# alebeck/jax-raft

Hardware: AMD Instinct MI355X
Metric: image-pairs/sec + Sintel-clean EPE, raft_large 32 iters at 1/2/4/8 MI355X (higher is better)
Workload: dtype bf16

## Files before the change

csrc/kernels/gru_fused.hip:

```cpp
#include <cstdlib>

#include "conv_igemm.h"

namespace {

constexpr int HD = 128;
constexpr int CIN = 256;
constexpr int KPAD = 5 * CIN;
constexpr int NSTG = KPAD / BK;
constexpr int AROWS = 2 * HD;
constexpr int ASTAGE = AROWS * BK;
constexpr int IMG_ROWS = 136;
constexpr unsigned OOB = 0x80000000u;
static_assert(2 * HD * BK + 128 * HD <= 2 * ASTAGE, "G2ALL: GEMM 2 buffers + the z image fit GEMM 1's staging");

JR_DEVICE int rh_off(int row, int chunk) { return row * HD + ((chunk ^ (row & 15)) << 3); }
JR_DEVICE int img_off(int row, int chunk) { return row * CIN + ((chunk ^ (row & 15)) << 3); }

template <int NV>
JR_DEVICE void load_map(const GruFusedParams& p, int m, int c, float* v) {
  const long o = (long)m * p.bmap_cs + c;
  if (p.bmap_bf16) load_bf16<NV>((const bf16*)p.bmap + o, v);
  else load_f32<NV>((const float*)p.bmap + o, v);
}

template <bool G2ALL>
__global__ __launch_bounds__(1024) void gru_fused_kernel(const GruFusedParams p) {
  __shared__ __attribute__((aligned(16))) bf16 smem[2 * ASTAGE + IMG_ROWS * CIN];
  bf16* const img = smem + 2 * ASTAGE;

  const int tid = threadIdx.x, lane = tid & 63, wave = tid >> 6;
  const int wco = wave & 3, wp = wave >> 2;
  const int rho = lane & 31, hh = lane >> 5;
  const int tile = blockIdx.x;
  auto stamp = [&](int k) {
    if (p.dbg && tid == 0) p.dbg[tile * 6 + k] = (long long)wall_clock64();
  };
  stamp(0);
  const int n = tile / p.tiles_per_img, tt = tile - n * p.tiles_per_img;
  const int npx = p.J * p.L;
  auto pix = [&](int pl) -> int {
    if (pl >= npx) return -1;
    const int j = pl / p.L, r = pl - j * p.L;
    const int y = p.vertical ? r : tt;
    const int x = p.vertical ? tt * p.J + j : r;
    return (n * p.H + y) * p.W + x;
  };

  const __amdgpu_buffer_rsrc_t xs = __builtin_amdgcn_make_buffer_rsrc((void*)p.hx, (short)0, (int)p.hx_bytes, 0x00020000);
  const __amdgpu_buffer_rsrc_t was = __builtin_amdgcn_make_buffer_rsrc((void*)p.wa, (short)0, (int)p.wa_bytes, 0x00020000);
  const __amdgpu_buffer_rsrc_t wbs = __builtin_amdgcn_make_buffer_rsrc((void*)p.wb, (short)0, (int)p.wb_bytes, 0x00020000);

  const int lrow = tid >> 3, ch = tid & 7;
  const unsigned aoff = (unsigned)(lrow * KPAD * 2 + ch * 16);
  auto kofs = [&](int s) { return (unsigned)((s >> 2) * CIN + (s & 3) * 64) * 2u; };
  auto sA_of = [&](int buf) { return smem + buf * ASTAGE; };
  auto putA = [&](bf16* base, int row, const u32x4& v) { *(u32x4*)(base + row * BK + ((ch ^ swzA(row)) << 3)) = v; };

  constexpr int NIMG = (IMG_ROWS * 32 + 1023) / 1024;
  u32x4 iv[NIMG];
  const int nrow = p.J * (p.L + 4);
#pragma unroll
  for (int k = 0; k < NIMG; ++k) {
    const int idx = k * 1024 + tid, R = idx >> 5, c = idx & 31;
    const int j = R / (p.L + 4), r = R - j * (p.L + 4) - 2;
    const bool in = R < nrow && (unsigned)r < (unsigned)p.L;
    const int m = in ? pix(j * p.L + r) : 0;
    iv[k] = __builtin_bit_cast(u32x4, __builtin_amdgcn_raw_buffer_load_b128(
        xs, in ? (unsigned)m * (unsigned)p.hx_cs * 2u + (unsigned)c * 16u : OOB, 0, 0));
  }

  struct Regs { u32x4 a0, a1; };
  auto issue1 = [&](Regs& r, int s) {
    const bool kin = s < NSTG;
    r.a0 = __builtin_bit_cast(u32x4, __builtin_amdgcn_raw_buffer_load_b128(was, kin ? aoff + kofs(s) : OOB, 0, 0));
    r.a1 = __builtin_bit_cast(u32x4, __builtin_amdgcn_raw_buffer_load_b128(
        was, kin ? aoff + (unsigned)(128 * KPAD * 2) + kofs(s) : OOB, 0, 0));
  };
  auto store1 = [&](const Regs& r, int buf) {
    putA(sA_of(buf), lrow, r.a0);
    putA(sA_of(buf), lrow + 128, r.a1);
  };
  f32x16 acc[2];
#pragma unroll
  for (int t = 0; t < 2; ++t)
#pragma unroll
    for (int k = 0; k < 16; ++k) acc[t][k] = 0.f;
  const int prow = wp * 32 + rho;
  const int m = pix(prow);
  const int jrun = prow / p.L;
  const int rh_row = prow < npx ? jrun * (p.L + 4) + (prow - jrun * p.L) : 0;
  auto bimg = [&](int s, int chunk) {
    const int row = rh_row + (s >> 2);
    return *(const bf16x8*)(img + img_off(row, (s & 3) * 8 + chunk));
  };
  const int mld = m >= 0 ? m : 0;
  auto pre_map = [&](u32x4 (&r)[2], int c) {
    const u32x4* q = (const u32x4*)((const bf16*)p.bmap + (long)mld * p.bmap_cs + c);
    r[0] = q[0];
    r[1] = q[1];
  };
  auto map16 = [&](const u32x4 (&r)[2], int c, float* v) {
    if (p.bmap_bf16) {
#pragma unroll
      for (int k = 0; k < 8; ++k) {
        v[k] = bf2f(__builtin_bit_cast(bf16x8, r[0])[k]);
        v[8 + k] = bf2f(__builtin_bit_cast(bf16x8, r[1])[k]);
      }
    } else {
      load_map<16>(p, m, c, v);
    }
  };
  auto mma_stage = [&](const bf16* sA, int arow0, int s) {
#pragma unroll
    for (int kk = 0; kk < 4; ++kk) {
      const int chunk = kk * 2 + hh;
      const bf16x8 b = bimg(s, chunk);
#pragma unroll
      for (int t = 0; t < 2; ++t) {
        const int row = arow0 + m32_arow(t, rho);
        const bf16x8 a = *(const bf16x8*)(sA + row * BK + ((chunk ^ swzA(row)) << 3));
        acc[t] = __builtin_amdgcn_mfma_f32_32x32x16_bf16(a, b, acc[t], 0, 0, 0);
      }
    }
  };
  u32x4 bm1[2][2];
  {
    Regs ra, rb;
    issue1(ra, 0);
    issue1(rb, 1);
#pragma unroll
    for (int k = 0; k < NIMG; ++k) {
      const int idx = k * 1024 + tid, R = idx >> 5, c = idx & 31;
      if (R < IMG_ROWS) *(u32x4*)(img + img_off(R, c)) = iv[k];
    }
    store1(ra, 0);
    __syncthreads();
#pragma nounroll
    for (int s = 0; s < NSTG - 2; s += 2) {
      issue1(ra, s + 2);
      mma_stage(sA_of(0), wco * 64, s);
      store1(rb, 1);
      __syncthreads();
      issue1(rb, s + 3);
      mma_stage(sA_of(1), wco * 64, s + 1);
      store1(ra, 0);
      __syncthreads();
    }
#pragma unroll
    for (int t = 0; t < 2; ++t) pre_map(bm1[t], wco * 64 + 32 * t + 16 * hh);
    mma_stage(sA_of(0), wco * 64, NSTG - 2);
    store1(rb, 1);
    __syncthreads();
    mma_stage(sA_of(1), wco * 64, NSTG - 1);
    __syncthreads();
  }

  stamp(1);
  auto sA2 = [&](int buf) { return smem + buf * (HD * BK); };
  auto issue2 = [&](u32x4& r, int s) {
    r = __builtin_bit_cast(u32x4, __builtin_amdgcn_raw_buffer_load_b128(wbs, s < NSTG ? aoff + kofs(s) : OOB, 0, 0));
  };
  u32x4 ra2, rb2;
  issue2(ra2, 0);
  issue2(rb2, 1);

  bf16* const zimg = smem + 2 * HD * BK;
  [[maybe_unused]] bf16x8 z[2][2];
#pragma unroll
  for (int t = 0; t < 2; ++t) {
// ... 100 lines not shown
    if constexpr (G2ALL) {
      zz[0] = *(const bf16x8*)(zimg + rh_off(prow, c0 >> 3));
      zz[1] = *(const bf16x8*)(zimg + rh_off(prow, (c0 >> 3) + 1));
    } else {
      zz[0] = z[t][0];
      zz[1] = z[t][1];
    }
    float b[16], h[16], v[16];
    map16(bm2[t], 2 * HD + c0, b);
    float* hp = p.h32 + (long)m * HD + c0;
    if constexpr (G2ALL) {
#pragma unroll
      for (int k = 0; k < 16; ++k) h[k] = h2[k >> 2][k & 3];
    } else {
      load_f32<16>(hp, h);
    }
#pragma unroll
    for (int k = 0; k < 16; ++k) {
      const float q = tanhf_(acc[t][k] + b[k]);
      const float zk = bf2f(zz[k >> 3][k & 7]);
      v[k] = (1.0f - zk) * h[k] + zk * q;
    }
    store_f32<16>(hp, v);
    store_bf16<16>((bf16*)p.y + (long)m * p.y_cs + c0, v);
    if (p.y2) store_bf16<16>((bf16*)p.y2 + (long)m * p.y2_cs + c0, v);
  }
  stamp(4);
}

}

extern "C" int jr_gru_fused(const GruFusedParams* p, hipStream_t stream) {
  if (p->ntiles <= 0) return 0;
  if (p->g2all) hipLaunchKernelGGL(gru_fused_kernel<true>, dim3(p->ntiles), dim3(1024), 0, stream, *p);
  else hipLaunchKernelGGL(gru_fused_kernel<false>, dim3(p->ntiles), dim3(1024), 0, stream, *p);
  return (int)hipGetLastError();
}
```

csrc/kernels/kernels.h:

```cpp
#pragma once
#include <hip/hip_runtime.h>
#include <stdint.h>

extern "C" {

enum ConvEpi : int {
  EPI_STD = 0,
  EPI_GRU_A = 1,
  EPI_GRU_B = 2,
  EPI_BWD = 5,
  EPI_TAPS = 6,
};

struct BwdSeg {
  int mode;
  const void* gin; int gin_cs, gin_coff, gin_bf16;
  const void* mask; int mask_cs, mask_coff;
  int valid;
  void* out; int out_cs, out_coff, out_f32;
};

struct ConvParams {
  const void* x;
  int N, H, W;
// ... 182 lines not shown
  int ksplit; float* part;
};
int jr_conv_f32(const ConvF32Params* p, int epi, hipStream_t stream);
int jr_channel_stats_f32(const float* x, int N, int HW, int C, float* stats, float* partial, hipStream_t stream);
int jr_norm_act_f32(const float* x, const float* sx, int mode_x, const float* res, const float* sr, int mode_r,
                    float* y, int N, int HW, int C, float eps, int relu, hipStream_t stream);
int jr_prep_images_f32(const float* img1, const float* img2, int B, int H, int W, float* out, hipStream_t stream);
int jr_copy_channels_f32(const float* src, int s_cstride, int s_coff, float* dst, int d_cstride, int d_coff, int M,
                         int C, hipStream_t stream);
int jr_upsample_convex_f32(const float* mask, int mask_cstride, const float* flow, int B, int h, int w, float* out,
                           const void* out_slot, long out_off, hipStream_t stream);
int jr_corr_pool_f32(const float* src, long M, int hl, int wl, float* dst, hipStream_t stream);
int jr_corr_lookup_f32(const float* const* levels, int num_levels, int B, int h, int w, int nq, int radius,
                       const float* coords, float* out, int out_cstride, hipStream_t stream);
int jr_flow_update_f32(const float* delta, int dcs, int N, int h, int w, float* coords, float* flow32, float* hx,
                       int hx_cs, int hx_off, float* qx, int qx_cs, int qx_off, float* flow4, hipStream_t stream);

struct GruFusedParams {
  const void* hx; int hx_cs;
  const void* wa; const void* wb;
  const void* bmap; int bmap_cs; int bmap_bf16;
  float* h32;
  void* y; int y_cs;
  void* y2; int y2_cs;
  int N, H, W;
  int vertical;
  int L, J, tiles_per_img, ntiles;
  int g2all;
  long hx_bytes, wa_bytes, wb_bytes;
  long long* dbg;
};
int jr_gru_fused(const GruFusedParams* p, hipStream_t stream);

struct GruHaloParams {
  const void* hsrc; const void* xsrc; int cs;
  const void* wa; const void* wb;
  const void* bmap; int bmap_cs;
  float* h32;
  void* y; int y_cs;
  void* y2; int y2_cs;
  int N, H, W;
  int mode;
  int axis;
  int TR, TC;
  int tiles_y, tiles_x, ntiles;
  int nb1, nb2;
  long src_bytes, wa_bytes, wb_bytes;
  const float* h32in;
  void* zo; void* ro; void* qo; void* rh; int rh_cs;
};
int jr_gru_halo(const GruHaloParams* p, hipStream_t stream);

int jr_gru_halo_lds(int hd, int mode, int TR, int TC, int nb1, int nb2);
struct ConvHaloParams {
  const void* x; int xcs, xoff;
  int N, H, W, cin;
  const void* w; long w_bytes;
  const float* bias; int cout;
  int act;
  void* y; int ycs, yoff;
  void* y2; int y2cs, y2off;
  const void* res; int rcs, roff, res_post;
  float* stats_part;
  const float* in_stats; int in_hw; float in_eps; int in_relu;
  const void* in_res; int in_rcs; const float* in_res_stats;
  void* xn; int xncs;
// ... 17 lines not shown
```

csrc/runtime/binding.cpp:

```cpp
#include <torch/custom_class.h>
#include <torch/library.h>
#include <ATen/ATen.h>
#include <c10/core/DeviceGuard.h>
#include <c10/hip/HIPStream.h>
#include <hip/hip_runtime.h>

#include <algorithm>
#include <array>
#include <functional>
#include <string>
#include <vector>

#include "../kernels/kernels.h"
#include "plan.h"

namespace jr {

using TList = c10::List<c10::optional<at::Tensor>>;
using IList = std::vector<int64_t>;

static inline at::Tensor opt(const TList& t, size_t i) {
  if (i >= t.size()) return at::Tensor();
  c10::optional<at::Tensor> v = t.get(i);
  return v.has_value() ? *v : at::Tensor();
// ... 531 lines not shown

static Launch make_conv1x1(const TList& t, const IList& i, std::vector<at::Tensor>& keep) {
  at::Tensor x = opt(t, 0), wpk = opt(t, 1), bias = opt(t, 2), y = opt(t, 3);
  check_bf16(x, "x"); check_bf16(wpk, "wpk"); check_f32(bias, "bias"); check_bf16(y, "y");
  const int64_t M = i[0];
  const int kvalid = (int)i[1], kpad = (int)i[2], cout = (int)i[3], act = (int)i[4], ycoff = (int)i[5];
  TORCH_CHECK(cout % 64 == 0 && kpad % 32 == 0 && kvalid <= kpad && kvalid % 8 == 0 && kvalid <= cs(x),
              "conv1x1: shapes");
  TORCH_CHECK(cs(x) % 8 == 0 && x.numel() >= M * cs(x) && reinterpret_cast<uintptr_t>(x.data_ptr()) % 16 == 0,
              "conv1x1: x [M][cs], 16-byte rows");
  TORCH_CHECK(wpk.numel() == (int64_t)cout * kpad && reinterpret_cast<uintptr_t>(wpk.data_ptr()) % 16 == 0,
              "conv1x1: packed weights (pack_conv1x1)");
  TORCH_CHECK(bias.numel() >= cout && reinterpret_cast<uintptr_t>(bias.data_ptr()) % 16 == 0, "conv1x1: bias");
  TORCH_CHECK(cs(y) % 8 == 0 && ycoff % 8 == 0 && ycoff + cout <= cs(y) && y.numel() >= M * cs(y) &&
                  reinterpret_cast<uintptr_t>(y.data_ptr()) % 16 == 0,
              "conv1x1: y [M][cs] with a 16-byte aligned cout-channel slice");
  keep.push_back(x); keep.push_back(wpk); keep.push_back(bias); keep.push_back(y);
  const void* xp = x.data_ptr();
  const void* wp = wpk.data_ptr();
  const float* bp = bias.data_ptr<float>();
  void* yp = y.data_ptr();
  const int xcs = cs(x), ycs = cs(y);
  return [=](hipStream_t s, int) {
    return jr_conv1x1_lds(xp, xcs, kvalid, kpad, wp, bp, act, yp, ycs, ycoff, cout, (int)M, s);
  };
}

bool gru_fused_fits(int64_t H, int64_t W, int64_t vertical) {
  if (!vertical) return W >= 1 && W <= 128;
  const int J = 2 * H <= 128 && W % 2 == 0 ? 2 : 1;
  return H >= 1 && J * H <= 128 && J * (H + 4) <= 136 && W % J == 0;
}

static Launch make_gru_fused(const TList& t, const IList& i, std::vector<at::Tensor>& keep) {
  at::Tensor hx = opt(t, 0), wa = opt(t, 1), wb = opt(t, 2), bmap = opt(t, 3), h32 = opt(t, 4), y = opt(t, 5),
             y2 = opt(t, 6), dbg = opt(t, 7);
  check_bf16(hx, "hx"); check_bf16(wa, "wa"); check_bf16(wb, "wb"); check_f32(h32, "h32"); check_bf16(y, "y");
  GruFusedParams p{};
  p.N = (int)i[0]; p.H = (int)i[1]; p.W = (int)i[2]; p.vertical = (int)i[3];
  p.g2all = i.size() == 5 ? (int)(i[4] != 0) : 1;
  const int64_t M = (int64_t)p.N * p.H * p.W;
  TORCH_CHECK(gru_fused_fits(p.H, p.W, p.vertical), "gru_fused: the tile geometry does not fit (", p.H, "x", p.W, ")");
  TORCH_CHECK(cs(hx) == 256 && hx.numel() >= M * 256 && reinterpret_cast<uintptr_t>(hx.data_ptr()) % 16 == 0,
              "gru_fused: hx must be [M][256] ([h 128 | x 128])");
  TORCH_CHECK(wa.numel() == 256 * 1280 && wb.numel() == 128 * 1280 &&
                  reinterpret_cast<uintptr_t>(wa.data_ptr()) % 16 == 0 && reinterpret_cast<uintptr_t>(wb.data_ptr()) % 16 == 0,
              "gru_fused: packed weights [256][1280] / [128][1280]");
  TORCH_CHECK(bmap.defined() && bmap.is_cuda() && bmap.is_contiguous() &&
                  (bmap.scalar_type() == at::kFloat || bmap.scalar_type() == at::kBFloat16) && cs(bmap) >= 384 &&
                  cs(bmap) % 8 == 0 && bmap.numel() >= M * cs(bmap) && reinterpret_cast<uintptr_t>(bmap.data_ptr()) % 16 == 0,
              "gru_fused: bias map [M][>=384] fp32 / bf16");
  TORCH_CHECK(h32.numel() >= M * 128 && cs(h32) == 128 && reinterpret_cast<uintptr_t>(h32.data_ptr()) % 16 == 0,
              "gru_fused: h32 [M][128]");
  TORCH_CHECK(cs(y) % 8 == 0 && cs(y) >= 128 && y.numel() >= M * cs(y) && reinterpret_cast<uintptr_t>(y.data_ptr()) % 16 == 0,
              "gru_fused: y [M][>=128]");
  if (y2.defined()) {
    check_bf16(y2, "y2");
    TORCH_CHECK(cs(y2) % 8 == 0 && cs(y2) >= 128 && y2.numel() >= M * cs(y2) &&
                    reinterpret_cast<uintptr_t>(y2.data_ptr()) % 16 == 0, "gru_fused: y2 [M][>=128]");
  }
  p.hx = hx.data_ptr(); p.hx_cs = 256; p.wa = wa.data_ptr(); p.wb = wb.data_ptr();
  p.bmap = bmap.data_ptr(); p.bmap_cs = cs(bmap); p.bmap_bf16 = bmap.scalar_type() == at::kBFloat16;
  p.h32 = h32.data_ptr<float>(); p.y = y.data_ptr(); p.y_cs = cs(y); p.y2 = ptr(y2); p.y2_cs = y2.defined() ? cs(y2) : 0;
  if (!p.vertical) { p.L = p.W; p.J = 1; p.tiles_per_img = p.H; }
  else { p.L = p.H; p.J = 2 * p.H <= 128 && p.W % 2 == 0 ? 2 : 1; p.tiles_per_img = p.W / p.J; }
  p.ntiles = p.N * p.tiles_per_img;
  if (dbg.defined()) {
    TORCH_CHECK(dbg.is_cuda() && dbg.scalar_type() == at::kLong && dbg.numel() >= (int64_t)p.ntiles * 6, "gru_fused: dbg");
    p.dbg = (long long*)dbg.data_ptr();
  }
  p.hx_bytes = (long)hx.numel() * 2; p.wa_bytes = (long)wa.numel() * 2; p.wb_bytes = (long)wb.numel() * 2;
  TORCH_CHECK(p.hx_bytes < (1LL << 31), "gru_fused: hx larger than 2 GiB");
  for (auto& v : {hx, wa, wb, bmap, h32, y, y2}) if (v.defined()) keep.push_back(v);
  at::Tensor y2b = opt(t, 8);
  if (y2b.defined()) {
    TORCH_CHECK(y2.defined(), "gru_fused: an odd-iteration y2 needs y2");
    check_bf16(y2b, "y2 (odd)");
    TORCH_CHECK(y2b.sizes() == y2.sizes() && reinterpret_cast<uintptr_t>(y2b.data_ptr()) % 16 == 0,
                "gru_fused: odd-iteration y2 must have y2's shape");
    GruFusedParams q = p;
    q.y2 = y2b.data_ptr();
    keep.push_back(y2b);
    return [p, q](hipStream_t s, int it) { return jr_gru_fused((it & 1) ? &q : &p, s); };
  }
  return [p](hipStream_t s, int) { return jr_gru_fused(&p, s); };
}

bool gru_halo_geom_ok(int64_t hd, int64_t mode, int64_t TR, int64_t TC, int64_t nb1, int64_t nb2) {
  if (TR < 1 || TC < 1) return false;
  const int64_t nreg = mode == 0 ? TC + 4 : (TR + 2) * (TC + 2);
  const int64_t nout = TR * TC;
  if ((mode == 0 && (TR != 1 || hd != 128)) || (mode == 1 && hd != 96) || mode < 0 || mode > 1) return false;
  if (nreg > 32 * nb1 || nout > 32 * nb2) return false;
  return jr_gru_halo_lds((int)hd, (int)mode, (int)TR, (int)TC, (int)nb1, (int)nb2) > 0 &&
         jr_gru_halo_lds((int)hd, (int)mode, (int)TR, (int)TC, (int)nb1, (int)nb2) <= 160 * 1024;
}

static Launch make_gru_halo(const TList& t, const IList& i, std::vector<at::Tensor>& keep) {
  at::Tensor hs = opt(t, 0), xs = opt(t, 1), wa = opt(t, 2), wb = opt(t, 3), bmap = opt(t, 4), h32 = opt(t, 5),
             y = opt(t, 6), y2 = opt(t, 7);
  check_bf16(hs, "hsrc"); check_bf16(xs, "xsrc"); check_bf16(wa, "wa"); check_bf16(wb, "wb"); check_bf16(bmap, "bmap");
  check_f32(h32, "h32"); check_bf16(y, "y");
  GruHaloParams p{};
  p.N = (int)i[0]; p.H = (int)i[1]; p.W = (int)i[2]; p.mode = (int)i[3]; p.axis = (int)i[4];
  p.TR = (int)i[5]; p.TC = (int)i[6]; p.nb1 = (int)i[7]; p.nb2 = (int)i[8];
  const int64_t M = (int64_t)p.N * p.H * p.W;
  const int cs_ = cs(hs), hd = cs_ / 2;
  const int taps = p.mode == 0 ? 5 : 9;
  TORCH_CHECK(p.N >= 1 && p.H >= 1 && p.W >= 1 && M < (1LL << 31), "gru_halo: map size");
  TORCH_CHECK(gru_halo_geom_ok(hd, p.mode, p.TR, p.TC, p.nb1, p.nb2), "gru_halo: unsupported tile (hd ", hd, ", mode ",
              p.mode, ", ", p.TR, "x", p.TC, ", blocks ", p.nb1, "/", p.nb2, ")");
  TORCH_CHECK(p.mode == 1 || p.axis == 0 || p.axis == 1, "gru_halo: axis must be 0 (1x5) or 1 (5x1)");
  TORCH_CHECK(cs(xs) == cs_ && hs.numel() >= M * cs_ && xs.numel() >= M * cs_ && hs.numel() == xs.numel(),
              "gru_halo: hsrc / xsrc must be [M][2 hd] with one shape");
  TORCH_CHECK(hs.data_ptr() != y.data_ptr(), "gru_halo: y must not alias hsrc (neighbouring tiles read h)");
  TORCH_CHECK(wa.numel() == (int64_t)2 * hd * taps * cs_ && wb.numel() == (int64_t)hd * taps * cs_,
              "gru_halo: packed weights (pack_gru_halo) of [z | r] and q");
  TORCH_CHECK(cs(bmap) >= 3 * hd && cs(bmap) % 8 == 0 && bmap.numel() >= M * cs(bmap), "gru_halo: bias map [M][>= 3 hd]");
// ... 1342 lines not shown
}
static Launch make_conv_fwd(const TList& t, const IList& i, double alpha, Keep& keep) { return make_conv(t, i, alpha, keep); }
static Launch make_init_flow_bf16(const TList& t, const IList& i, Keep& keep) { return make_init_flow(t, i, false, keep); }
static Launch make_init_flow_f32(const TList& t, const IList& i, Keep& keep) { return make_init_flow(t, i, true, keep); }

static const std::vector<OpRow>& op_table() {
  static const std::vector<OpRow> rows = {
      row_tia("conv", "alpha", 22, 29, make_conv_fwd),
      row_tia("corr", "scale", 5, 7, make_corr),
      row_ti("lookup", 5, 9, make_lookup, 1),
      row_ti("feat_pool", 5, 5, make_feat_pool),
      row_ti("lookup_od", 6, 8, make_lookup_od, 1),
      row_ti("upsample_convex", 4, 4, make_upsample_convex),
      row_tia("convex_head", "alpha", 5, 7, make_convex_head),
      row_ti("upsample_bilinear", 4, 5, make_upsample_bilinear),
      row_ti("stats", 3, 3, make_stats),
      row_ti("stats_final", 3, 3, make_stats_final),
      row_tia("norm_act", "eps", 6, 6, make_norm_act),
      row_ti("prep", 3, 8, make_prep),
      row_ti("init_coords", 3, 3, make_init_coords),
      row_ti("init_flow", 5, 5, make_init_flow_bf16),
      row_ti("init_flow_f32", 5, 5, make_init_flow_f32),
      row_ti("forward_project", 4, 4, make_forward_project),
      row_ti("fb_check", 7, 9, make_fb_check),
      row_ti("warp_frames", 8, 10, make_warp_frames),
      row_t("memset", make_memset),
      row_t("copy", make_copy),
      row_ti("copy_channels", 4, 4, make_copy_channels),
      row_ti("sum_iters", 2, 2, make_sum_iters),
      row_ti("im2col", 11, 11, make_im2col),
      row_ti("flow_taps", 5, 5, make_flow_taps),
      row_ti("taps_gemm", 3, 3, make_taps_gemm),
      row_ti("gru_fused", 4, 5, make_gru_fused),
      row_ti("gru_halo", 9, 9, make_gru_halo),
      row_ti("conv1x1", 6, 6, make_conv1x1),
      row_ti("conv_direct", 11, 11, make_conv_direct),
      row_tia("flowin_dual", "alpha", 15, 21, make_flowin_dual),
      row_tia("upsample_convex_bwd", "alpha", 3, 3, make_upsample_convex_bwd),
      row_ti("upsample_bilinear_bwd", 3, 3, make_upsample_bilinear_bwd),
      row_ti("flow_gather_bwd", 3, 3, make_flow_gather_bwd),
      row_ti("lookup_bwd", 5, 6, make_lookup_bwd),
      row_tia("norm_bwd", "eps", 5, 5, make_norm_bwd),
      row_ti("pack", 2, 2, make_pack),
      row_ti("wgrad", 16, 16, make_wgrad),
      row_ti("bn_table", 2, 2, make_bn_table),
      row_ti("augment_sums", 3, 3, make_augment_sums),
      row_ti("augment", 5, 5, make_augment),
      row_ti("augment_sparse_sums", 3, 3, make_augment_sparse_sums),
      row_ti("augment_sparse", 5, 5, make_augment_sparse),
      row_ti("augment_mixed_sums", 2, 2, make_augment_mixed_sums),
      row_ti("augment_mixed", 4, 4, make_augment_mixed),
      row_ti("flow_metrics", 6, 6, make_flow_metrics),
      row_tia("conv_f32", "alpha", 22, 22, make_conv_f32),
      row_ti("stats_f32", 3, 3, make_stats_f32),
      row_tia("norm_act_f32", "eps", 6, 6, make_norm_act_f32),
      row_ti("prep_f32", 3, 3, make_prep_f32),
      row_ti("copy_channels_f32", 4, 4, make_copy_channels_f32),
      row_ti("upsample_convex_f32", 4, 5, make_upsample_convex_f32),
      row_ti("corr_pool_f32", 3, 3, make_corr_pool_f32),
      row_ti("lookup_f32", 5, 6, make_lookup_f32),
      row_ti("flow_update_f32", 5, 5, make_flow_update_f32),
  };
  return rows;
}

std::vector<int64_t> op_arity(std::string name) {
// ... 101 lines not shown
```

jax_raft_amd/runtime/engine.py:

```python
from __future__ import annotations

import itertools
import operator
import weakref
from collections import OrderedDict
from dataclasses import dataclass, field
from typing import Dict, List, Optional, Tuple

import torch

from ..models.reference import BidirectionalFlow, BidirectionalWarp
from ..models.layers import (
    NORM_BATCH,
    NORM_CUSTOM,
    NORM_INSTANCE,
    BottleneckBlock,
    ConvNormActivation,
    CorrBlock,
    FeatureEncoder,
    FlowHead,
    MaskPredictor,
    MotionEncoder,
    RecurrentBlock,
    ResidualBlock,
# ... 100 lines not shown
    ph = (((H0 // 8) + 1) * 8 - H0) % 8
    pw = (((W0 // 8) + 1) * 8 - W0) % 8
    return ph // 2, ph - ph // 2, pw // 2, pw - pw // 2


_U8_LUT: Dict[str, torch.Tensor] = {}


def u8_table(device) -> torch.Tensor:
    key = str(device)
    t = _U8_LUT.get(key)
    if t is None:
        t = _U8_LUT[key] = (torch.arange(256, dtype=torch.float32) / 255.0 * 2.0 - 1.0).to(device)
    return t


class RaftEngine:

    def __new__(cls, *args, precision: str = "bf16", **kwargs):
        if precision not in ("bf16", "fp32", "mixed"):
            raise ValueError(f"precision must be 'bf16', 'fp32' or 'mixed', got {precision!r}")
        if precision == "fp32" and cls is RaftEngine:
            from .engine_f32 import RaftEngineF32
            cls = RaftEngineF32
        elif precision == "mixed" and cls is RaftEngine:
            from .engine_f32 import RaftEngineMixed
            cls = RaftEngineMixed
        return super().__new__(cls)

    precision = "bf16"
    fe_external = False

    GRU = "auto"
    PRO_LANES = "auto"
    HALO_NORM = True
    MERGED_UP = True
    CONV_GROUP = True
    MASK_PARITY = False
    CORR_PERSIST_B1 = True
    HOST_GATE = True
    WARM_FILL_RADIUS = 4

    def __init__(self, model, device, use_graph: bool = True, copy_output: bool = True,
                 corr_dtype: torch.dtype = torch.bfloat16, gate_dtype: torch.dtype = torch.bfloat16,
                 autotune: bool = True, streams="auto", split: int = 1,
                 cfg_override: Optional[Dict[str, int]] = None, cp_group=None, **mode):
        mode.pop("precision", None)
        corr = mode.pop("corr", "volume")
        if mode:
            raise TypeError(f"RaftEngine: unexpected keyword arguments {sorted(mode)}")
        if corr not in ("volume", "on_demand"):
            raise ValueError(f"corr must be 'volume' or 'on_demand', got {corr!r}")
        if corr == "on_demand":
            if self.precision != "bf16":
                raise NotImplementedError(f"corr='on_demand': not with precision={self.precision!r} (the on-demand "
                                          "lookup is lowered for the bf16 engine only)")
            if cp_group is not None:
                raise NotImplementedError("corr='on_demand': not with context parallelism (cp_group splits the "
                                          "volume the on-demand path never builds)")
        self.corr_mode = corr
        nat.require()
        self._init_cp(cp_group)
        assert streams in (True, False, "auto"), streams
        self.streams_mode = streams
        self.streams = bool(streams)
        self.halo_norm = bool(self.HALO_NORM)
# ... 646 lines not shown
        if code is None:
            code = tunedb.lookup(self.arch, key, set(enc))
        if code is None:
            t, base = ops_args
            best = None
            for c, tile in enc.items():
                nat.ops().gru_halo(t, base + list(tile))
                s_, e_ = torch.cuda.Event(enable_timing=True), torch.cuda.Event(enable_timing=True)
                s_.record()
                for _ in range(5):
                    nat.ops().gru_halo(t, base + list(tile))
                e_.record()
                e_.synchronize()
                el = s_.elapsed_time(e_)
                if best is None or el < best[0]:
                    best = (el, c)
            code = best[1]
            tunedb.record(self.arch, key, code)
        code = self._agree(code)
        _TUNE_CACHE[key + (str(self.device),)] = code
        self.chosen_cfgs[f"gru{gi}.halo"] = code
        return enc[code]

    def _gru_fused_ok(self, B: int, h: int, w: int) -> bool:
        env = "1" if self.GRU == "fused" else "auto"
        rb = self.model.update_block.recurrent_block
        ks = [tuple(k) for k in rb.kernel_size]
        if (self.hidden != 128 or self.hx_cs != 256 or self.gate_cs < 384 or ks != [(1, 5), (5, 1)]
                or self.gate_dtype != torch.bfloat16):
            return False
        tiles = min(nat.gru_fused_tiles(B, h, w, 0), nat.gru_fused_tiles(B, h, w, 1))
        return tiles > 0 and (env == "1" or tiles >= 3 * nat.NUM_CUS // 4)

    def uses_lanes(self, B: int, all_iters: bool = True) -> bool:
        if self.cp or not self._lanes_ok(all_iters):
            return False
        if self.streams_mode != "auto":
            return bool(self.streams_mode)
        nb = B // self.split if (self.split > 1 and B % self.split == 0) else B
        return nb >= self.AUTO_STREAMS_MIN_BATCH

    def _build(self, B: int, H: int, W: int, n_iters: int, all_iters: bool = True,
               src: Optional[Tuple[int, int, int, int]] = None, warm: bool = False) -> _PlanState:
        if warm and self.cp:
            raise NotImplementedError("warm start (flow_init) is not lowered under context parallelism")
        parts = self.split if (self.split > 1 and B % self.split == 0 and not self.cp) else 1
        nb = B // parts
        st, lanes = self._new_state(B, H, W, n_iters, all_iters, src, self.uses_lanes(B, all_iters), parts, B)
        if warm:
            st.flow_init = torch.zeros((B, H // 8, W // 8, 2), dtype=F32, device=self.device)
        for part, plan in enumerate(st.plans):
            self._build_part(st, plan, part * nb, nb, H, W, n_iters, f"p{part}.", lanes, 0, all_iters, warm)
            plan.set_lane(0)
            plan.set_segment(2)
        return st

    def _new_state(self, B: int, H: int, W: int, n_iters: int, all_iters: bool,
                   src: Optional[Tuple[int, int, int, int]], on: bool, parts: int, out_batch: int):
        self.streams = on
        self.mask_head = "split" if on else "fused"
        h, w = H // 8, W // 8
        min_sz = 2 * (2 ** (self.num_levels - 1))
        assert h >= min_sz and w >= min_sz, (
            f"Feature maps are too small to be down-sampled by the correlation pyramid: need >= {min_sz}, got {(h, w)}; "
            f"input images should be at least {8 * min_sz}.")
        dev = self.device
# ... 169 lines not shown
            plan.add_feat_pool([fmap[Bi:]] + pooled, [Bi, h, w, self.fmap_ch, L])
        elif self.cp:
            for b in range(B):
                plan.add_corr([fmap[b, r0:r1], fmap[B + b]] + [v[b * nq:(b + 1) * nq] for v in levels] + [None] * (4 - L),
                              [1, h, w, self.fmap_ch, L, nq, 0], scale)
        else:
            bl = 2 if (blocked and self.CORR_PERSIST_B1 and not getattr(self, "_slot_build", False)) else blocked
            plan.add_corr([fmap[:Bi], fmap[Bi:]] + levels + [None] * (4 - L), [Bi, h, w, self.fmap_ch, L, h * w, bl],
                          scale)
            if bidir:
                plan.add_corr([fmap[Bi:], fmap[:Bi]] + [v[Bi * h * w:] for v in levels] + [None] * (4 - L),
                              [Bi, h, w, self.fmap_ch, L, h * w, bl], scale)
        plan.add_wait(E_CTX)

        me = m.update_block.motion_encoder
        cl, fl = me.corr_layers, me.flow_layers
        corr = alloc("corr", (M, self.corr_cs))
        cf = alloc("cf", (M, cl[-1] + fl[-1]))
        f1 = alloc("f1", (M, fl[0]))
        c1 = alloc("c1", (M, cl[0])) if len(cl) == 2 else None
        taps = alloc("fh2.taps", (M, 24), F32)
        stride = st.out.shape[1] * H * W * 2
        split_mask = lanes_on or self.cp
        s1 = sp["fh1"] if (self.has_mask and all_iters and not split_mask) else sp["fh1.flow"] if self.has_mask else sp["fh1"]
        taps_epi = self._taps_epi_w is not None and s1.cout == 256
        fm = None if taps_epi else alloc("fm", (M, round_up(s1.cout, 8)))
        mfeat = (alloc("mfeat", (M, round_up(sp["mask.convrelu"].cout, 8)))
                 if self.has_mask and (split_mask or not all_iters) else None)
        mask = alloc("mask", (M, 576)) if self.has_mask and self._convex_w is None else None
        gru_path = self._gru_path(B, h, w)
        if gru_path == "fused" and self.cp:
            gru_path = "unfused"
        self.gru_path = gru_path
        ngru = len(m.update_block.recurrent_block.kernel_size)
        halo_pp = gru_path == "halo" and ngru == 1
        qx_x = gru_path != "halo" or halo_pp
        hm = (alloc("hm", (M, self.hidden))
              if gru_path != "unfused" and self.has_mask and (lanes_on or halo_pp) else None)
        parity = (hm is not None and gru_path == "fused" and self._convex_w is not None
                  and self.MASK_PARITY)
        hm2 = alloc("hm2", (M, self.hidden)) if parity else None
        flow32b = alloc("flow32b", (M, 2), F32) if parity else None
        st.flow_out.append((b0, B, flow32, flow32b))

        c1k = me.convflow1.layers_0.kernel
        merged_up = (self._cf1_w is not None and tuple(c1k.shape[:2]) == (7, 7) and not self.cp
                     and (not self.has_mask or (self._convex_w is not None and fm is not None))
                     and self.MERGED_UP)

        def flow_features():
            if self._cf1_w is not None:
                c = me.convflow1.layers_0
                kh, kw_, _, co = c.kernel.shape
                plan.add_conv_direct([flow8, self._cf1_w, self._cf1_b, f1],
                                     [B, h, w, 2, kh, kw_, c.padding[0], c.padding[1], co, 1, 0])
            else:
                self._conv(plan, sp["me.convflow1"], flow8, B, h, w, f1, act=ACT_RELU)
            self._conv(plan, sp["me.convflow2"], f1, B, h, w, cf, y_coff=cl[-1], act=ACT_RELU)

        def flow_head():
            if taps_epi:
                self._conv(plan, s1, hx, B, h, w, taps, act=ACT_RELU, epi=EPI_TAPS, tapw=self._taps_epi_w)
                return
            if halo_pp:
                self._conv(plan, s1, qx, B, h, w, fm, x_alt=hx, act=ACT_RELU)
            else:
# ... 30 lines not shown
            upd = [taps, self._fh2_b, flow32, hx, qx if qx_x else None, flow8] if with_update else []
            if with_update and parity:
                upd.append(flow32b)
            extra = [self.flow_off, self.flow_off] if with_update else []
            if on_demand:
                plan.add_lookup_od([coords, corr, fmap[:Bi], fmap[Bi:]] + pooled + [None] * (4 - L) + upd,
                                   [L, B, h, w, self.radius, self.fmap_ch] + extra)
                return
            plan.add_lookup([coords, corr] + levels + [None] * (4 - L) + upd,
                            [L, B, h, w, self.radius, h * w, blocked] + extra)

        c1_merged = (merged_up and self.has_mask and len(cl) == 2 and self._cc1_w is not None
                     and self._cc1_kpad == 352)

        def motion_and_gru(wait_flow: bool, wait_mask: bool, flow2: bool = False):
            if len(cl) == 2:
                if flow2 and c1_merged:
                    pass
                elif self._cc1_w is not None:
                    plan.add_conv1x1([corr, self._cc1_w, self._cc1_b, c1],
                                     [M, self.corr_cs, self._cc1_kpad, cl[0], ACT_RELU, 0])
                else:
                    self._conv(plan, sp["me.convcorr1"], corr, B, h, w, c1, act=ACT_RELU)
                last = (sp["me.convcorr2"], c1, B, h, w, cf, dict(act=ACT_RELU))
            else:
                last = (sp["me.convcorr1"], corr, B, h, w, cf, dict(act=ACT_RELU))
            fl2 = (sp["me.convflow2"], f1, B, h, w, cf, dict(y_coff=cl[-1], act=ACT_RELU))
            if not (flow2 and self.CONV_GROUP and self._conv_group(plan, last, fl2)):
                if flow2:
                    self._conv(plan, *fl2[:6], **fl2[6])
                self._conv(plan, *last[:6], **last[6])
            if wait_flow:
                plan.add_wait(E_FLOW)
            self._conv(plan, sp["me.conv"], cf, B, h, w, hx, y_coff=self.mot_off, act=ACT_RELU,
                       y2=qx if qx_x else None, y2_coff=self.mot_off)
            if gru_path == "halo":
                _, stages = self._halo_geom()
                for gi, (mode, axis) in enumerate(stages):
                    wa_, wb_ = self._halo_w[gi]
                    last = gi == ngru - 1
                    if halo_pp:
                        t = [hx, hx, wa_, wb_, gbias[gi], h32, qx, hm, qx, qx, hx]
                    else:
                        t = [hx if gi == 0 else qx, hx, wa_, wb_, gbias[gi], h32, qx if gi == 0 else hx,
                             hm if last else None]
                    if wait_mask and last:
                        plan.add_wait(E_MASK)
                    base = [B, h, w, mode, axis]
                    tile = self._halo_tile(gi, mode, axis, B, h, w, (t, base))
                    plan.add_gru_halo(t, base + list(tile))
                return
            for gi in range(ngru):
                if gru_path == "fused":
                    last = gi == ngru - 1
                    if wait_mask and not parity and (last if hm is not None else gi == 0):
                        plan.add_wait(E_MASK)
                    ks = m.update_block.recurrent_block.kernel_size[gi]
                    plan.add_gru_fused([hx, sp[f"gru{gi}.a"].w, sp[f"gru{gi}.b"].w, gbias[gi], h32, hx,
                                        hm if last else None] + ([None, hm2] if last and parity else []),
                                       [B, h, w, int(ks[0] > 1)])
                    continue
                self._conv(plan, sp[f"gru{gi}.a"], hx, B, h, w, qx, zbuf=zb, hidden=self.hidden,
                           epi=EPI_GRU_A, bmap=gbias[gi], bmap_coff=0)
                if gi == 0 and wait_mask:
                    plan.add_wait(E_MASK)
                self._conv(plan, sp[f"gru{gi}.b"], qx, B, h, w, hx, h32=h32, zbuf=zb, hidden=self.hidden,
                           epi=EPI_GRU_B, bmap=gbias[gi], bmap_coff=2 * self.hidden)

        if self.cp:
            hw = h * w
            local = alloc("corr.local", (B, max(b_ - a_ for a_, b_ in slabs) * w, self.corr_cs))
            plan.set_segment(1)
            for b in range(B):
                plan.add_lookup([coords[b * hw + r0 * w:b * hw + r1 * w], local[b]]
                                + [v[b * nq:(b + 1) * nq] for v in levels] + [None] * (4 - L),
                                [L, 1, h, w, self.radius, nq, 0])
            plan.set_segment(3)
            flow_features()
            motion_and_gru(wait_flow=False, wait_mask=False)
            flow_head()
            flow_update()
            if all_iters:
                upsample(stride, mask_from_fm=False)
            plan.set_segment(2)
            if not all_iters:
                upsample(0, mask_from_fm=False)
            st.cp = dict(slabs=slabs, local=local, corr=corr, w=w)
        elif lanes_on:
            plan.set_segment(0)
            lane(main)
# ... 321 lines not shown
```

Baseline: 422.0.

## Fuse motion-encoder 3x3 conv into the first fused GRU kernel

Adds a templated ME variant of the fused GRU kernel that computes the motion-encoder 3x3 conv (256->cout, ReLU) per row tile from the correlation/flow features in shared memory. The result is written into hx and straight into the LDS image used by the GRU's first GEMM, which removes a separate conv launch and the round trip of those features through global memory. The engine picks this path automatically when the geometry fits (horizontal first stage, width up to 128, enough tiles). The trade-off is a longer serial prologue in each GRU block, and every tile recomputes the 3x3 conv on its own rows, so occupancy and overlap with other work may change.

```diff
diff --git a/csrc/kernels/gru_fused.hip b/csrc/kernels/gru_fused.hip
--- a/csrc/kernels/gru_fused.hip
+++ b/csrc/kernels/gru_fused.hip
@@ -1,4 +1,5 @@
 #include <cstdlib>
+#include <type_traits>
 
 #include "conv_igemm.h"
 
@@ -24,8 +25,12 @@
   else load_f32<NV>((const float*)p.bmap + o, v);
 }
 
-template <bool G2ALL>
-__global__ __launch_bounds__(1024) void gru_fused_kernel(const GruFusedParams p) {
+template <bool G2ALL, bool ME = false>
+__global__ __launch_bounds__(1024) void gru_fused_kernel(const std::conditional_t<ME, GruFusedMeParams, GruFusedParams> pp) {
+  const GruFusedParams& p = [&]() -> const GruFusedParams& {
+    if constexpr (ME) return pp.g;
+    else return pp;
+  }();
   __shared__ __attribute__((aligned(16))) bf16 smem[2 * ASTAGE + IMG_ROWS * CIN];
   bf16* const img = smem + 2 * ASTAGE;
 
@@ -34,7 +39,7 @@
   const int rho = lane & 31, hh = lane >> 5;
   const int tile = blockIdx.x;
   auto stamp = [&](int k) {
-    if (p.dbg && tid == 0) p.dbg[tile * 6 + k] = (long long)wall_clock64();
+    if (p.dbg && tid == 0) p.dbg[tile * (ME ? 8 : 6) + k] = (long long)wall_clock64();
   };
   stamp(0);
   const int n = tile / p.tiles_per_img, tt = tile - n * p.tiles_per_img;
@@ -58,10 +63,10 @@
   auto putA = [&](bf16* base, int row, const u32x4& v) { *(u32x4*)(base + row * BK + ((ch ^ swzA(row)) << 3)) = v; };
 
   constexpr int NIMG = (IMG_ROWS * 32 + 1023) / 1024;
-  u32x4 iv[NIMG];
+  [[maybe_unused]] u32x4 iv[NIMG];
   const int nrow = p.J * (p.L + 4);
 #pragma unroll
-  for (int k = 0; k < NIMG; ++k) {
+  for (int k = 0; k < (ME ? 0 : NIMG); ++k) {
     const int idx = k * 1024 + tid, R = idx >> 5, c = idx & 31;
     const int j = R / (p.L + 4), r = R - j * (p.L + 4) - 2;
     const bool in = R < nrow && (unsigned)r < (unsigned)p.L;
@@ -82,10 +87,6 @@
     putA(sA_of(buf), lrow + 128, r.a1);
   };
   f32x16 acc[2];
-#pragma unroll
-  for (int t = 0; t < 2; ++t)
-#pragma unroll
-    for (int k = 0; k < 16; ++k) acc[t][k] = 0.f;
   const int prow = wp * 32 + rho;
   const int m = pix(prow);
   const int jrun = prow / p.L;
@@ -125,17 +126,165 @@
     }
   };
   u32x4 bm1[2][2];
-  {
-    Regs ra, rb;
+  Regs ra, rb;
+  if constexpr (ME) {
+    constexpr int KME = 9 * CIN, NSME = KME / BK, CF_ROWS = 130;
+    constexpr int NCF = (CF_ROWS * 32 + 1023) / 1024;
+    constexpr int NHI = (IMG_ROWS * 16 + 1023) / 1024;
+    const __amdgpu_buffer_rsrc_t cfs = __builtin_amdgcn_make_buffer_rsrc((void*)pp.cf, (short)0, (int)pp.cf_bytes, 0x00020000);
+    const __amdgpu_buffer_rsrc_t wms = __builtin_amdgcn_make_buffer_rsrc((void*)pp.wm, (short)0, (int)pp.wm_bytes, 0x00020000);
+    const unsigned moff = (unsigned)(lrow * KME * 2 + ch * 16);
+    auto issueM = [&](u32x4& r, int s) {
+      r = __builtin_bit_cast(u32x4, __builtin_amdgcn_raw_buffer_load_b128(wms, s < NSME ? moff + (unsigned)s * (BK * 2u) : OOB, 0, 0));
+    };
+    auto sAm = [&](int buf) { return smem + buf * (HD * BK); };
+    u32x4 cv[NCF];
+    auto cfload = [&](int u) {
+      const int yy = tt + u - 1;
+      const bool yin = (unsigned)yy < (unsigned)p.H;
+#pragma unroll
+      for (int k = 0; k < NCF; ++k) {
+        const int idx = k * 1024 + tid, R = idx >> 5, c = idx & 31;
+        const bool in = yin && (unsigned)(R - 1) < (unsigned)p.W;
+        const int mm = (n * p.H + yy) * p.W + R - 1;
+        cv[k] = __builtin_bit_cast(u32x4, __builtin_amdgcn_raw_buffer_load_b128(
+            cfs, in ? (unsigned)mm * (unsigned)pp.cf_cs * 2u + (unsigned)c * 16u : OOB, 0, 0));
+      }
+    };
+    auto cfstore = [&]() {
+#pragma unroll
+      for (int k = 0; k < NCF; ++k) {
+        const int idx = k * 1024 + tid, R = idx >> 5, c = idx & 31;
+        if (R < CF_ROWS) *(u32x4*)(img + img_off(R, c)) = cv[k];
+      }
+    };
+    const int prowM = (wave >> 2) * 32 + rho;
+    const int arowM = 64 * (wco >> 1) + m32_arow(wco & 1, rho);
+    f32x16 accm;
+#pragma unroll
+    for (int k = 0; k < 16; ++k) accm[k] = 0.f;
+    auto computeM = [&](int buf, int j) {
+      const bf16* sA = sAm(buf);
+      const int row = prowM + (j >> 2);
+#pragma unroll
+      for (int kk = 0; kk < 4; ++kk) {
+        const int chunk = kk * 2 + hh;
+        const bf16x8 b = *(const bf16x8*)(img + img_off(row, (j & 3) * 8 + chunk));
+        const bf16x8 a = *(const bf16x8*)(sA + arowM * BK + ((chunk ^ swzA(arowM)) << 3));
+        accm = __builtin_amdgcn_mfma_f32_32x32x16_bf16(a, b, accm, 0, 0, 0);
+      }
+    };
+    float* const bl = (float*)(smem + 2 * HD * BK);
+    const float bias_t = pp.bias[(tid & (HD - 1)) < pp.cout ? (tid & (HD - 1)) : pp.cout - 1];
+    u32x4 ma, mb;
+    cfload(0);
+    issueM(ma, 0);
+    issueM(mb, 1);
+    cfstore();
+    if (tid < HD) bl[tid] = bias_t;
+    cfload(1);
+    putA(sAm(0), lrow, ma);
+    __syncthreads();
+    stamp(6);
+#pragma unroll
+    for (int u = 0; u < 3; ++u) {
+      const int jend = u == 2 ? 10 : 12;
+#pragma nounroll
+      for (int j = 0; j < jend; j += 2) {
+        issueM(ma, u * 12 + j + 2);
+        computeM(0, j);
+        putA(sAm(1), lrow, mb);
+        __syncthreads();
+        issueM(mb, u * 12 + j + 3);
+        computeM(1, j + 1);
+        putA(sAm(0), lrow, ma);
+        __syncthreads();
+      }
+      if (u < 2) {
+        cfstore();
+        if (u == 0) cfload(2);
+        __syncthreads();
+      }
+    }
+    const int mM = pix(prowM), mldM = mM >= 0 ? mM : 0;
+    const int c0 = 32 * wco + 16 * hh;
+    u32x4 xh[2];
+    {
+      const u32x4* q = (const u32x4*)((const bf16*)p.hx + (long)mldM * p.hx_cs + HD + c0);
+      xh[0] = q[0];
+      xh[1] = q[1];
+    }
+    u32x4 hv[NHI];
+#pragma unroll
+    for (int k = 0; k < NHI; ++k) {
+      const int idx = k * 1024 + tid, R = idx >> 4, c = idx & 15;
+      const bool in = R < nrow && (unsigned)(R - 2) < (unsigned)p.L;
+      const int mm = in ? pix(R - 2) : 0;
+      hv[k] = __builtin_bit_cast(u32x4, __builtin_amdgcn_raw_buffer_load_b128(
+          xs, in ? (unsigned)mm * (unsigned)p.hx_cs * 2u + (unsigned)c * 16u : OOB, 0, 0));
+    }
     issue1(ra, 0);
     issue1(rb, 1);
-#pragma unroll
-    for (int k = 0; k < NIMG; ++k) {
-      const int idx = k * 1024 + tid, R = idx >> 5, c = idx & 31;
-      if (R < IMG_ROWS) *(u32x4*)(img + img_off(R, c)) = iv[k];
+    computeM(0, 10);
+    putA(sAm(1), lrow, mb);
+    __syncthreads();
+    computeM(1, 11);
+    __syncthreads();
+    float bv[16];
+#pragma unroll
+    for (int k = 0; k < 4; ++k) *(f32x4*)(bv + 4 * k) = *(const f32x4*)(bl + c0 + 4 * k);
+    bf16x8 o[2];
+#pragma unroll
+    for (int k = 0; k < 16; ++k) {
+      const bf16 keep = __builtin_bit_cast(bf16x8, xh[k >> 3])[k & 7];
+      o[k >> 3][k & 7] = c0 + k < pp.cout ? f2bf(fmaxf(accm[k] + bv[k], 0.f)) : keep;
+    }
+    if (mM < 0) {
+#pragma unroll
+      for (int k = 0; k < 16; ++k) o[k >> 3][k & 7] = f2bf(0.f);
+    } else {
+      bf16* yp = (bf16*)p.hx + (long)mM * p.hx_cs + HD + c0;
+#pragma unroll
+      for (int q = 0; q < 2; ++q) {
+        if (c0 + 8 * q + 8 <= pp.cout) {
+          *(bf16x8*)(yp + 8 * q) = o[q];
+        } else {
+#pragma unroll
+          for (int k = 0; k < 8; ++k)
+            if (c0 + 8 * q + k < pp.cout) yp[8 * q + k] = o[q][k];
+        }
+      }
+    }
+    *(bf16x8*)(img + img_off(prowM + 2, 16 + (c0 >> 3))) = o[0];
+    *(bf16x8*)(img + img_off(prowM + 2, 17 + (c0 >> 3))) = o[1];
+    if (tid < 128) {
+      const int R = tid >> 4;
+      const u32x4 zero = {0u, 0u, 0u, 0u};
+      *(u32x4*)(img + img_off(R < 2 ? R : 128 + R, 16 + (tid & 15))) = zero;
+    }
+#pragma unroll
+    for (int k = 0; k < NHI; ++k) {
+      const int idx = k * 1024 + tid, R = idx >> 4, c = idx & 15;
+      if (R < IMG_ROWS) *(u32x4*)(img + img_off(R, c)) = hv[k];
+    }
+  }
+#pragma unroll
+  for (int t = 0; t < 2; ++t)
+#pragma unroll
+    for (int k = 0; k < 16; ++k) acc[t][k] = 0.f;
+  {
+    if constexpr (!ME) {
+      issue1(ra, 0);
+      issue1(rb, 1);
+#pragma unroll
+      for (int k = 0; k < NIMG; ++k) {
+        const int idx = k * 1024 + tid, R = idx >> 5, c = idx & 31;
+        if (R < IMG_ROWS) *(u32x4*)(img + img_off(R, c)) = iv[k];
+      }
     }
     store1(ra, 0);
     __syncthreads();
+    stamp(5);
 #pragma nounroll
     for (int s = 0; s < NSTG - 2; s += 2) {
       issue1(ra, s + 2);
@@ -302,7 +451,14 @@
 
 extern "C" int jr_gru_fused(const GruFusedParams* p, hipStream_t stream) {
   if (p->ntiles <= 0) return 0;
-  if (p->g2all) hipLaunchKernelGGL(gru_fused_kernel<true>, dim3(p->ntiles), dim3(1024), 0, stream, *p);
-  else hipLaunchKernelGGL(gru_fused_kernel<false>, dim3(p->ntiles), dim3(1024), 0, stream, *p);
+  if (p->g2all) hipLaunchKernelGGL((gru_fused_kernel<true>), dim3(p->ntiles), dim3(1024), 0, stream, *p);
+  else hipLaunchKernelGGL((gru_fused_kernel<false>), dim3(p->ntiles), dim3(1024), 0, stream, *p);
   return (int)hipGetLastError();
 }
+
+extern "C" int jr_gru_fused_me(const GruFusedMeParams* p, hipStream_t stream) {
+  if (p->g.ntiles <= 0) return 0;
+  if (p->g.vertical || !p->g.g2all || p->g.J != 1 || p->cout < 1 || p->cout > HD) return (int)hipErrorInvalidValue;
+  hipLaunchKernelGGL((gru_fused_kernel<true, true>), dim3(p->g.ntiles), dim3(1024), 0, stream, *p);
+  return (int)hipGetLastError();
+}
diff --git a/csrc/kernels/kernels.h b/csrc/kernels/kernels.h
--- a/csrc/kernels/kernels.h
+++ b/csrc/kernels/kernels.h
@@ -238,6 +238,16 @@
 };
 int jr_gru_fused(const GruFusedParams* p, hipStream_t stream);
 
+struct GruFusedMeParams {
+  GruFusedParams g;
+  const void* cf; int cf_cs;
+  const void* wm;
+  const float* bias;
+  int cout;
+  long cf_bytes, wm_bytes;
+};
+int jr_gru_fused_me(const GruFusedMeParams* p, hipStream_t stream);
+
 struct GruHaloParams {
   const void* hsrc; const void* xsrc; int cs;
   const void* wa; const void* wb;
diff --git a/csrc/runtime/binding.cpp b/csrc/runtime/binding.cpp
--- a/csrc/runtime/binding.cpp
+++ b/csrc/runtime/binding.cpp
@@ -587,13 +587,14 @@
   return H >= 1 && J * H <= 128 && J * (H + 4) <= 136 && W % J == 0;
 }
 
-static Launch make_gru_fused(const TList& t, const IList& i, std::vector<at::Tensor>& keep) {
+static GruFusedParams gru_fused_params(const TList& t, int N, int H, int W, int vertical, int g2all, int dbg_slots,
+                                       std::vector<at::Tensor>& keep) {
   at::Tensor hx = opt(t, 0), wa = opt(t, 1), wb = opt(t, 2), bmap = opt(t, 3), h32 = opt(t, 4), y = opt(t, 5),
              y2 = opt(t, 6), dbg = opt(t, 7);
   check_bf16(hx, "hx"); check_bf16(wa, "wa"); check_bf16(wb, "wb"); check_f32(h32, "h32"); check_bf16(y, "y");
   GruFusedParams p{};
-  p.N = (int)i[0]; p.H = (int)i[1]; p.W = (int)i[2]; p.vertical = (int)i[3];
-  p.g2all = i.size() == 5 ? (int)(i[4] != 0) : 1;
+  p.N = N; p.H = H; p.W = W; p.vertical = vertical;
+  p.g2all = g2all;
   const int64_t M = (int64_t)p.N * p.H * p.W;
   TORCH_CHECK(gru_fused_fits(p.H, p.W, p.vertical), "gru_fused: the tile geometry does not fit (", p.H, "x", p.W, ")");
   TORCH_CHECK(cs(hx) == 256 && hx.numel() >= M * 256 && reinterpret_cast<uintptr_t>(hx.data_ptr()) % 16 == 0,
@@ -621,12 +622,19 @@
   else { p.L = p.H; p.J = 2 * p.H <= 128 && p.W % 2 == 0 ? 2 : 1; p.tiles_per_img = p.W / p.J; }
   p.ntiles = p.N * p.tiles_per_img;
   if (dbg.defined()) {
-    TORCH_CHECK(dbg.is_cuda() && dbg.scalar_type() == at::kLong && dbg.numel() >= (int64_t)p.ntiles * 6, "gru_fused: dbg");
+    TORCH_CHECK(dbg.is_cuda() && dbg.scalar_type() == at::kLong && dbg.numel() >= (int64_t)p.ntiles * dbg_slots, "gru_fused: dbg");
     p.dbg = (long long*)dbg.data_ptr();
   }
   p.hx_bytes = (long)hx.numel() * 2; p.wa_bytes = (long)wa.numel() * 2; p.wb_bytes = (long)wb.numel() * 2;
   TORCH_CHECK(p.hx_bytes < (1LL << 31), "gru_fused: hx larger than 2 GiB");
   for (auto& v : {hx, wa, wb, bmap, h32, y, y2}) if (v.defined()) keep.push_back(v);
+  return p;
+}
+
+static Launch make_gru_fused(const TList& t, const IList& i, std::vector<at::Tensor>& keep) {
+  const GruFusedParams p = gru_fused_params(t, (int)i[0], (int)i[1], (int)i[2], (int)i[3],
+                                            i.size() == 5 ? (int)(i[4] != 0) : 1, 6, keep);
+  at::Tensor y2 = opt(t, 6);
   at::Tensor y2b = opt(t, 8);
   if (y2b.defined()) {
     TORCH_CHECK(y2.defined(), "gru_fused: an odd-iteration y2 needs y2");
@@ -639,6 +647,26 @@
     return [p, q](hipStream_t s, int it) { return jr_gru_fused((it & 1) ? &q : &p, s); };
   }
   return [p](hipStream_t s, int) { return jr_gru_fused(&p, s); };
+}
+
+static Launch make_gru_fused_me(const TList& t, const IList& i, std::vector<at::Tensor>& keep) {
+  GruFusedMeParams p{};
+  p.g = gru_fused_params(t, (int)i[0], (int)i[1], (int)i[2], 0, 1, 8, keep);
+  at::Tensor cf = opt(t, 8), wm = opt(t, 9), bias = opt(t, 10);
+  check_bf16(cf, "cf"); check_bf16(wm, "wm"); check_f32(bias, "bias");
+  p.cout = (int)i[3];
+  const int64_t M = (int64_t)p.g.N * p.g.H * p.g.W;
+  TORCH_CHECK(p.cout >= 1 && p.cout <= 128 && bias.numel() >= p.cout, "gru_fused_me: 1 .. 128 output channels with a bias each");
+  TORCH_CHECK(cs(cf) >= 256 && cs(cf) % 8 == 0 && cf.numel() >= M * cs(cf) && reinterpret_cast<uintptr_t>(cf.data_ptr()) % 16 == 0,
+              "gru_fused_me: cf must be [M][>=256]");
+  TORCH_CHECK(wm.numel() == 128 * 2304 && reinterpret_cast<uintptr_t>(wm.data_ptr()) % 16 == 0,
+              "gru_fused_me: packed 3x3 weights [128][2304]");
+  TORCH_CHECK(p.g.y == p.g.hx, "gru_fused_me: the stage runs in place (y is hx)");
+  p.cf = cf.data_ptr(); p.cf_cs = cs(cf); p.wm = wm.data_ptr(); p.bias = bias.data_ptr<float>();
+  p.cf_bytes = (long)cf.numel() * 2; p.wm_bytes = (long)wm.numel() * 2;
+  TORCH_CHECK(p.cf_bytes < (1LL << 31), "gru_fused_me: cf larger than 2 GiB");
+  keep.push_back(cf); keep.push_back(wm); keep.push_back(bias);
+  return [p](hipStream_t s, int) { return jr_gru_fused_me(&p, s); };
 }
 
 bool gru_halo_geom_ok(int64_t hd, int64_t mode, int64_t TR, int64_t TC, int64_t nb1, int64_t nb2) {
@@ -2047,6 +2075,7 @@
       row_ti("flow_taps", 5, 5, make_flow_taps),
       row_ti("taps_gemm", 3, 3, make_taps_gemm),
       row_ti("gru_fused", 4, 5, make_gru_fused),
+      row_ti("gru_fused_me", 4, 4, make_gru_fused_me),
       row_ti("gru_halo", 9, 9, make_gru_halo),
       row_ti("conv1x1", 6, 6, make_conv1x1),
       row_ti("conv_direct", 11, 11, make_conv_direct),
diff --git a/jax_raft_amd/runtime/engine.py b/jax_raft_amd/runtime/engine.py
--- a/jax_raft_amd/runtime/engine.py
+++ b/jax_raft_amd/runtime/engine.py
@@ -156,6 +156,7 @@
     fe_external = False
 
     GRU = "auto"
+    GRU_ME = "auto"
     PRO_LANES = "auto"
     HALO_NORM = True
     MERGED_UP = True
@@ -868,6 +869,17 @@
         tiles = min(nat.gru_fused_tiles(B, h, w, 0), nat.gru_fused_tiles(B, h, w, 1))
         return tiles > 0 and (env == "1" or tiles >= 3 * nat.NUM_CUS // 4)
 
+    def _gru_me_ok(self, B: int, h: int, w: int) -> bool:
+        assert self.GRU_ME in ("auto", "on", "off"), self.GRU_ME
+        if self.GRU_ME == "off" or self.cp:
+            return False
+        sp = self._specs["me.conv"]
+        ks = tuple(self.model.update_block.recurrent_block.kernel_size[0])
+        if (not (sp.halo_ks == 3 and sp.cin8 == 256 and sp.cout <= 128 and self.mot_off == 128 and self.hx_cs == 256)
+                or ks != (1, 5) or not 1 <= w <= 128):
+            return False
+        return self.GRU_ME == "on" or nat.gru_fused_tiles(B, h, w, 0) >= 3 * nat.NUM_CUS // 4
+
     def uses_lanes(self, B: int, all_iters: bool = True) -> bool:
         if self.cp or not self._lanes_ok(all_iters):
             return False
@@ -1103,6 +1115,7 @@
         if gru_path == "fused" and self.cp:
             gru_path = "unfused"
         self.gru_path = gru_path
+        gru_me = gru_path == "fused" and self._gru_me_ok(B, h, w)
         ngru = len(m.update_block.recurrent_block.kernel_size)
         halo_pp = gru_path == "halo" and ngru == 1
         qx_x = gru_path != "halo" or halo_pp
@@ -1199,8 +1212,9 @@
                 self._conv(plan, *last[:6], **last[6])
             if wait_flow:
                 plan.add_wait(E_FLOW)
-            self._conv(plan, sp["me.conv"], cf, B, h, w, hx, y_coff=self.mot_off, act=ACT_RELU,
-                       y2=qx if qx_x else None, y2_coff=self.mot_off)
+            if not gru_me:
+                self._conv(plan, sp["me.conv"], cf, B, h, w, hx, y_coff=self.mot_off, act=ACT_RELU,
+                           y2=qx if qx_x else None, y2_coff=self.mot_off)
             if gru_path == "halo":
                 _, stages = self._halo_geom()
                 for gi, (mode, axis) in enumerate(stages):
@@ -1223,6 +1237,11 @@
                     if wait_mask and not parity and (last if hm is not None else gi == 0):
                         plan.add_wait(E_MASK)
                     ks = m.update_block.recurrent_block.kernel_size[gi]
+                    if gi == 0 and gru_me:
+                        mc = sp["me.conv"]
+                        plan.add_gru_fused_me([hx, sp["gru0.a"].w, sp["gru0.b"].w, gbias[0], h32, hx,
+                                               hm if last else None, None, cf, mc.w, mc.b], [B, h, w, mc.cout])
+                        continue
                     plan.add_gru_fused([hx, sp[f"gru{gi}.a"].w, sp[f"gru{gi}.b"].w, gbias[gi], h32, hx,
                                         hm if last else None] + ([None, hm2] if last and parity else []),
                                        [B, h, w, int(ks[0] > 1)])
```

After: 427.8, median of 6. 1.01x the previous value.
